# virajmehta/vae-training

Measured on AMD Instinct MI355X. Metric: ELBO train-step samples/sec, higher is better.
Workload: dtype f32; 1 GPU; M: linear-padding dd3 pad9 (D=12) L=20 linear enc/dec -tdv eps=-1 lr=1e-3 (seed_linpadding_expts.sh:1); batch_per_gpu=65536, global_batch=65536, data_dim=12, latent_dim=20, params=533, parallelism=dp1, grad_exchange=none, launch=direct library call x2395 steps (arguments marshalled once), input_batches=48

## Files before the change

vae_training_amd/csrc/linear_moments.hip:

```cpp
#include <stdlib.h>

#include <type_traits>

#include "comm_dev.h"
#include "rng_dev.h"
#include "vaek_internal.h"

namespace vaek {

using f32x4 = __attribute__((ext_vector_type(4))) float;
using d2 = __attribute__((ext_vector_type(2))) double;
typedef __attribute__((address_space(3))) void lds_void_t;
typedef const __attribute__((address_space(1))) void glb_void_t;

constexpr int LNT = 512, LNW = LNT / 64;
constexpr int kLinMaxPersist = 64;
constexpr int kLinReduceSets = 1;
constexpr int kLinReduceWgs = 24;

constexpr int kLinCommBanks = 4;
struct LinComm { unsigned long long* peer[kMaxWorld]; int world, rank, ng2; };

constexpr int kLinShards = 8, kLinShardStride = 32;
struct LinPtrs { const float* x[64]; const float* z1[64]; const float* z2[64]; };
struct LinArgs {
    int has_update, n_reduce, n_stream;
    int B, D, L, ntiles, T;
    const float* x; const float* z1; const float* z2; float* partial_out;
    const float* partial_in; double* M_out;
    const double* M_in;
    int persistent, n_steps, sets;
    float* partial_base; double* M_base;
    unsigned* cnt_stream; unsigned* cnt_reduce; unsigned* status;
    float* params; float* grads; float* m; float* v; int32_t* step_dev; float lr;
    float inv_bt, eps_cli, rows, rows_over_bt; int off_eps, P;
    float* loss_hist; long long loss_hist_cap;
    int stagger;
    LinComm comm;
};

#ifndef VAEK_LIN_ABL
#define VAEK_LIN_ABL 0
#endif
#ifdef VAEK_LIN_STAMPS
#ifdef VAEK_LIN_FOUR_BLOCK_TU
static __device__ unsigned long long* g_lin_stamp_buf = nullptr;
#else
__device__ unsigned long long* g_lin_stamp_buf = nullptr;
#endif
int lin_stamps_four(unsigned long long* buf);
#define LIN_STAMP(i)                                                                                         \
    do {                                                                                                     \
        if (VAEK_LIN_STAMPS == 2) break;          \
        __builtin_amdgcn_sched_barrier(0);                                                                   \
        unsigned long long _t;                                                                               \
        unsigned long long _r;                                                                               \
        asm volatile("s_waitcnt vmcnt(0) lgkmcnt(0)\n\ts_memtime %0\n\ts_memrealtime %1\n\ts_waitcnt lgkmcnt(0)" : "=s"(_t), "=s"(_r)::"memory"); \
        if (g_lin_stamp_buf && threadIdx.x == 0) { g_lin_stamp_buf[i] = _t; g_lin_stamp_buf[16 + (i)] = _r; } \
        __builtin_amdgcn_sched_barrier(0);                                                                   \
    } while (0)
#define LIN_NOW(v)                                                                                           \
    do {                                                                                                     \
        __builtin_amdgcn_sched_barrier(0);                                                                   \
        if (VAEK_LIN_STAMPS == 2) asm volatile("s_memrealtime %0\n\ts_waitcnt lgkmcnt(0)" : "=s"(v)::"memory");             \
        else asm volatile("s_waitcnt vmcnt(0) lgkmcnt(0)\n\ts_memrealtime %0\n\ts_waitcnt lgkmcnt(0)" : "=s"(v)::"memory"); \
        __builtin_amdgcn_sched_barrier(0);                                                                   \
    } while (0)
#define LIN_NOWQ(v)                                     \
    do {                                                                                                     \
        __builtin_amdgcn_sched_barrier(0);                                                                   \
        asm volatile("s_memrealtime %0\n\ts_waitcnt lgkmcnt(0)" : "=s"(v)::"memory");                        \
        __builtin_amdgcn_sched_barrier(0);                                                                   \
    } while (0)
#define LIN_PUT(i, v) do { if (g_lin_stamp_buf && threadIdx.x == 0) g_lin_stamp_buf[i] = (v); } while (0)
#define LIN_PUTMAX(i, v) do { if (g_lin_stamp_buf && threadIdx.x == 0) atomicMax(&g_lin_stamp_buf[i], (v)); } while (0)
#else
#define LIN_STAMP(i) do {} while (0)
#define LIN_NOW(v) do {} while (0)
#define LIN_NOWQ(v) do {} while (0)
#define LIN_PUT(i, v) do {} while (0)
#define LIN_PUTMAX(i, v) do {} while (0)
#endif

__device__ __forceinline__ void lin_glds16(const void* gsrc, void* lds_wave_base) {
    __builtin_amdgcn_global_load_lds((glb_void_t*)gsrc, (lds_void_t*)lds_wave_base, 16, 0, 0);
}
template <int N> __device__ __forceinline__ void lin_wait_vmcnt() { asm volatile("s_waitcnt vmcnt(%0)" ::"n"(N) : "memory"); }
__device__ __forceinline__ void lin_barrier() { asm volatile("s_waitcnt lgkmcnt(0)\n\ts_barrier" ::: "memory"); }
__device__ __forceinline__ void lin_wait_vmcnt_upto(int n) {
    switch (n) {
        case 1: lin_wait_vmcnt<1>(); break;   case 2: lin_wait_vmcnt<2>(); break;   case 3: lin_wait_vmcnt<3>(); break;
        case 4: lin_wait_vmcnt<4>(); break;   case 5: lin_wait_vmcnt<5>(); break;   case 6: lin_wait_vmcnt<6>(); break;
        case 7: lin_wait_vmcnt<7>(); break;   case 8: lin_wait_vmcnt<8>(); break;   case 9: lin_wait_vmcnt<9>(); break;
        case 10: lin_wait_vmcnt<10>(); break; case 11: lin_wait_vmcnt<11>(); break; case 12: lin_wait_vmcnt<12>(); break;
        case 13: lin_wait_vmcnt<13>(); break; case 14: lin_wait_vmcnt<14>(); break; case 15: lin_wait_vmcnt<15>(); break;
        case 16: lin_wait_vmcnt<16>(); break; case 17: lin_wait_vmcnt<17>(); break; case 18: lin_wait_vmcnt<18>(); break;
        case 19: lin_wait_vmcnt<19>(); break; case 20: lin_wait_vmcnt<20>(); break;
        default: lin_wait_vmcnt<0>(); break;
    }
}

__device__ __host__ constexpr int lin_blk(int NB, int b1, int b2) { return b1 * NB - b1 * (b1 - 1) / 2 + (b2 - b1); }

__device__ __forceinline__ void st_sc1(float* p, float v) { __hip_atomic_store(p, v, __ATOMIC_RELAXED, __HIP_MEMORY_SCOPE_AGENT); }
__device__ __forceinline__ void st_sc1(double* p, double v) { __hip_atomic_store(p, v, __ATOMIC_RELAXED, __HIP_MEMORY_SCOPE_AGENT); }
__device__ __forceinline__ float ld_sc1(const float* p) { return __hip_atomic_load(p, __ATOMIC_RELAXED, __HIP_MEMORY_SCOPE_AGENT); }
__device__ __forceinline__ double ld_sc1(const double* p) { return __hip_atomic_load(p, __ATOMIC_RELAXED, __HIP_MEMORY_SCOPE_AGENT); }

__device__ __forceinline__ void lin_wait_count(const unsigned* cnt, unsigned target, unsigned* status, unsigned tag) {
    if (threadIdx.x == 0) {
        unsigned spins = 0, seen;
        while ((seen = __hip_atomic_load(cnt, __ATOMIC_RELAXED, __HIP_MEMORY_SCOPE_AGENT)) < target) {
            __builtin_amdgcn_s_sleep(16);
            if ((++spins & 1023u) == 0) {
                if (__hip_atomic_load(status, __ATOMIC_RELAXED, __HIP_MEMORY_SCOPE_AGENT)) break;
                if (spins > (1u << 21)) {
                    unsigned expect = 0;
                    __hip_atomic_compare_exchange_strong(status, &expect, 0x80000000u | tag | (seen & 0xffffu), __ATOMIC_RELAXED,
                                                         __ATOMIC_RELAXED, __HIP_MEMORY_SCOPE_AGENT);
                    break;
                }
            }
        }
    }
    __syncthreads();
}

__device__ __forceinline__ void lin_wait_shards(const unsigned* cnt, unsigned target, unsigned* status, unsigned tag) {
    if (threadIdx.x == 0) {
        unsigned spins = 0, seen;
        for (;;) {
            unsigned v[kLinShards];
#pragma unroll
            for (int k = 0; k < kLinShards; ++k) v[k] = __hip_atomic_load(cnt + k * kLinShardStride, __ATOMIC_RELAXED, __HIP_MEMORY_SCOPE_AGENT);
            seen = 0;
#pragma unroll
            for (int k = 0; k < kLinShards; ++k) seen += v[k];
            if (seen >= target) break;
            __builtin_amdgcn_s_sleep(4);
            if ((++spins & 1023u) == 0) {
                if (__hip_atomic_load(status, __ATOMIC_RELAXED, __HIP_MEMORY_SCOPE_AGENT)) break;
                if (spins > (1u << 21)) {
                    unsigned expect = 0;
                    __hip_atomic_compare_exchange_strong(status, &expect, 0x80000000u | tag | (seen & 0xffffu), __ATOMIC_RELAXED,
                                                         __ATOMIC_RELAXED, __HIP_MEMORY_SCOPE_AGENT);
                    break;
                }
            }
        }
    }
    __syncthreads();
}

__device__ __forceinline__ double lin_sum_over_ranks(const LinComm& c, unsigned epoch, int o, double v, unsigned* status) {
    const unsigned long long bits = (unsigned long long)__double_as_longlong(v), tag = (unsigned long long)epoch << 32;
    const long long bank = (long long)(epoch & (kLinCommBanks - 1)) * c.world * c.ng2;
    for (int p = 0; p < c.world; ++p) {
        unsigned long long* q = c.peer[p] + bank + (long long)c.rank * c.ng2 + 2 * o;
        __hip_atomic_store(q, tag | (bits & 0xffffffffull), __ATOMIC_RELAXED, __HIP_MEMORY_SCOPE_SYSTEM);
        __hip_atomic_store(q + 1, tag | (bits >> 32), __ATOMIC_RELAXED, __HIP_MEMORY_SCOPE_SYSTEM);
    }
    const unsigned long long* own = c.peer[c.rank] + bank + 2 * o;
    double sum = 0.0;
    unsigned spins = 0;
    bool dead = false;
    for (int r = 0; r < c.world; ++r) {
        unsigned long long lo = 0, hi = 0;
        for (;;) {
            lo = __hip_atomic_load(own + (long long)r * c.ng2, __ATOMIC_RELAXED, __HIP_MEMORY_SCOPE_SYSTEM);
            hi = __hip_atomic_load(own + (long long)r * c.ng2 + 1, __ATOMIC_RELAXED, __HIP_MEMORY_SCOPE_SYSTEM);
            if (((unsigned)(lo >> 32) == epoch && (unsigned)(hi >> 32) == epoch) || dead) break;
            __builtin_amdgcn_s_sleep(8);
            if ((++spins & 1023u) == 0) {
                if (__hip_atomic_load(status, __ATOMIC_RELAXED, __HIP_MEMORY_SCOPE_AGENT)) dead = true;
                else if (spins > (1u << 21)) {
                    unsigned expect = 0;
                    __hip_atomic_compare_exchange_strong(status, &expect, 0x80000000u | (3u << 28) | ((unsigned)r << 16) | (epoch & 0xffffu),
                                                         __ATOMIC_RELAXED, __ATOMIC_RELAXED, __HIP_MEMORY_SCOPE_AGENT);
                    dead = true;
                }
            }
        }
        sum += __longlong_as_double((long long)((hi << 32) | (lo & 0xffffffffull)));
    }
// ... 1122 lines not shown
            double wsum = 0.0;
#pragma unroll
            for (int dt = 0; dt < PT; ++dt) {
                d4 C[2];
                double avk[KD], p1l[2][4], p1o[4], dw_sr[2], dw_br[2], dw_wr[KD][2], dw_dr[2][4];
                auto dw_s = [&](int ct) -> double& { return dw_sr[ct]; };
                auto dw_b = [&](int ct) -> double& { return dw_br[ct]; };
                auto dw_w = [&](int kk, int ct) -> double& { return dw_wr[kk][ct]; };
                auto dw_d = [&](int ct, int r) -> double& { return dw_dr[ct][r]; };
                const int d0 = 16 * dt;
#pragma unroll
                for (int ct = 0; ct < 2; ++ct) {
                    const int l = 16 * ct + j, lc = min(l, L - 1);
                    const double s_l = sd[lc], b_l = bed[lc];
                    dw_s(ct) = l < L ? s_l : 0.0; dw_b(ct) = l < L ? b_l : 0.0;
#pragma unroll
                    for (int kk = 0; kk < KD; ++kk) {
                        const int dd = 4 * kk + g;
                        const double w = Wed[min(dd, D - 1) * L + lc];
                        dw_w(kk, ct) = (dd < D && l < L) ? w : 0.0;
                    }
#pragma unroll
                    for (int r = 0; r < 4; ++r) dw_d(ct, r) = Wdd[lc * D + min(d0 + g + 4 * r, D - 1)];
                }
#pragma unroll
                for (int kk = 0; kk < KD; ++kk) avk[kk] = P1s[(d0 + j) * NFP + min(L + 4 * kk + g, NFP - 1)];
#pragma unroll
                for (int r = 0; r < 4; ++r) {
                    p1o[r] = P1s[(d0 + g + 4 * r) * NFP + fone];
#pragma unroll
                    for (int ct = 0; ct < 2; ++ct) p1l[ct][r] = P1s[(d0 + g + 4 * r) * NFP + min(16 * ct + j, L - 1)];
                }
                __builtin_amdgcn_sched_barrier(0);
#pragma unroll
                for (int ct = 0; ct < 2; ++ct) {
                    if (ct == 1 && RL1 == 0) continue;
                    const int l = 16 * ct + j;
#pragma unroll
                    for (int r = 0; r < 4; ++r) C[ct][r] = dw_s(ct) * p1l[ct][r] + dw_b(ct) * p1o[r];
#pragma unroll
                    for (int kk = 0; kk < KD; ++kk) C[ct] = __builtin_amdgcn_mfma_f64_16x16x4f64(avk[kk], dw_w(kk, ct), C[ct], 0, 0, 0);
#pragma unroll
                    for (int r = 0; r < 4; ++r) {
                        const int d = d0 + g + 4 * r;
                        if (l < L && d < D) { gq[off_wd + l * D + d] = c0 * C[ct][r]; wsum += dw_d(ct, r) * C[ct][r]; }
                    }
                }
            }
            wsum = lin_wave_sum(wsum);
            if (lane == 0) part[3 * NB] = wsum;
        }
        LIN_STAMP(4);
        __syncthreads();
        LIN_STAMP(5);
        const double rows = (double)a.rows;
        const float bc1 = (float)part[3 * NB + 4], bc2 = (float)part[3 * NB + 5];
#pragma unroll
        for (int k = 0; k < LKOUT; ++k) {
            const int idx = t + LNT * k;
            if (LNT * k >= P + 3) break;
            double gd = 0.0;
            if (idx < P && idx != off_eps) gd = gq[idx];
            else if (idx == off_eps || (idx >= P && idx < P + 3)) {
                double ssq = part[0], musq = part[1], z2r = part[2];
#pragma unroll
                for (int w = 1; w < NB; ++w) { ssq += part[3 * w]; musq += part[3 * w + 1]; z2r += part[3 * w + 2]; }
                ssq += part[3 * NB];
                const double klc = part[3 * NB + 3];
                if (idx == off_eps) gd = (double)a.eps_cli * (-0.5 * ssq * inv_var + 0.5 * rows * D + 0.5 * sigma * z2r * inv_var) * inv_bt;
                else {
                    const double dkl = (0.5 * musq - 0.5 * rows * klc) * inv_bt;
                    const double mse = (0.5 * ssq * inv_var + 0.5 * rows * D * ((double)kLog2Pi + eps)) * inv_bt;
                    gd = idx == P ? dkl + mse : (idx == P + 1 ? dkl : mse);
                }
            }
            const float gf = (float)gd;
            gout[k] = gf;
            if (idx == P && a.loss_hist) a.loss_hist[(long long)(tstep - 1) % a.loss_hist_cap] = gf;
            if (idx < P) adam_apply_f(pk(k), gf, mk(k), vk(k), a.lr, bc1, bc2);
        }
        LIN_STAMP(6);
    }
    __device__ __forceinline__ void store_state(const LinArgs& a, const float (&gout)[LKOUT], int tstep) {
        const int t = threadIdx.x;
#pragma unroll
        for (int k = 0; k < LKOUT; ++k) {
            const int idx = t + LNT * k;
            if (idx < P + kExtra) a.grads[idx] = gout[k];
            if (idx < P) { a.params[idx] = pk(k); a.m[idx] = mk(k); a.v[idx] = vk(k); }
        }
        if (t == 0) a.step_dev[0] = tstep;
    }
};

template <int NB, int DT, int LT>
using LinUpdMFor = std::conditional_t<NB == 3, LinUpdM<NB, DT, LT>, LinUpdMG<NB, DT, LT>>;

template <int NB, int DT, int LT>
__global__ __launch_bounds__(LNT) void lin_step_kernel(const LinArgs a) {
    extern __shared__ __attribute__((aligned(16))) char lin_smem[];
    const int b = blockIdx.x, t = threadIdx.x;
    constexpr int NO = NB * (NB + 1) / 2 * 256;
    if (b < a.has_update) {
        LinUpd<NB, DT, LT> u;
        u.carve(a, lin_smem);
        LIN_STAMP(0);
        const int tstep = a.step_dev[0] + 1;
        u.load_state(a);
        u.publish_params();
        u.template expand_M<false>(a.M_in);
        __syncthreads();
        float g[LKOUT];
        u.step(a, tstep, g);
        u.store_state(a, g, tstep);
        LIN_STAMP(7);
    } else if (b < a.has_update + a.n_reduce) {
        lin_reduce<false>(a.partial_in, a.M_out, a.ntiles, lin_smem, b - a.has_update, NO);
    } else {
        const int tile = b - a.has_update - a.n_reduce;
        const int wave = __builtin_amdgcn_readfirstlane(t >> 6), lane = t & 63;
        const LinTile tl(a.D, a.L, a.T);
        const int stride = max(tl.bytes, lin_scratch_bytes(NB)), v_off = stride, c_off = v_off + 4 * a.T;
        for (int p = wave; p < tl.np; p += LNW) lin_issue_piece(a, tl, a.x, a.z1, a.z2, tile, p, lin_smem, lane);
        lin_write_vcol(reinterpret_cast<float*>(lin_smem + v_off), a.T, (int)min((long long)a.T, (long long)a.B - (long long)tile * a.T), t);
        if (t == 0) *reinterpret_cast<float*>(lin_smem + c_off) = 0.f;
        lin_wait_vmcnt<0>();
        lin_barrier();
        lin_fix_ragged(a, tl, a.x, a.z1, a.z2, tile, lin_smem, t);
        f32x4 acc[NB * (NB + 1) / 2];
        lin_tile_products<NB, 0, LNW>(a, tl, lin_smem, 0, v_off, c_off, acc, lane, wave, [](int) {});
        lin_barrier();
        lin_tile_combine<NB, false, LNW>(acc, lin_smem, a.partial_out + (long long)tile * NO, t, wave, lane);
    }
}

template <int NB, int DT, int LT, int JT, bool GEN>
__global__ __launch_bounds__(LNT, 2) void lin_persist_kernel(const LinArgs a, const std::conditional_t<GEN, BatchArgs, LinPtrs> src) {
    extern __shared__ __attribute__((aligned(16))) char lin_smem[];
    const int b = blockIdx.x, t = threadIdx.x, N = a.n_steps;
    constexpr int NO = NB * (NB + 1) / 2 * 256;
    const int per_set = a.n_reduce / a.sets;
    if (b < a.has_update) {
        LinUpdMFor<NB, DT, LT> u;
        u.carve(a, lin_smem);
        int tstep = a.step_dev[0];
        u.load_state(a);
        float g[LKOUT];
#pragma unroll
        for (int k = 0; k < LKOUT; ++k) g[k] = 0.f;
        constexpr int NM = LinUpdMFor<NB, DT, LT>::NM;
        double mreg[NM], mnext[NM];
        bool have_next = false;
        LIN_STAMP(10);
        for (int n = 0; n < N; ++n) {
            LIN_STAMP(0);
            u.publish_params(a);
            LIN_STAMP(9);
            if (!have_next) {
                lin_wait_count(a.cnt_reduce + n, (unsigned)per_set, a.status, (1u << 28) | ((unsigned)n << 16));
                if (t < 64 * NB) u.fetch_M(a.M_base + (long long)n * NO, mreg);
            } else {
                __syncthreads();
#pragma unroll
                for (int k = 0; k < NM; ++k) mreg[k] = mnext[k];
            }
            LIN_STAMP(8);
            ++tstep;
            u.step(a, tstep, mreg, g, n + 1 < N ? a.cnt_reduce + n + 1 : nullptr, (unsigned)per_set, a.M_base + (long long)(n + 1) * NO, mnext, have_next);
            LIN_STAMP(7);
            { [[maybe_unused]] unsigned long long te = 0; LIN_NOWQ(te); LIN_PUT(64 + n, te); }
        }
        u.store_state(a, g, tstep);
        for (int k = t; k < N * kLinShards; k += LNT) __hip_atomic_store(a.cnt_stream + k * kLinShardStride, 0u, __ATOMIC_RELAXED, __HIP_MEMORY_SCOPE_AGENT);
        for (int k = t; k < N; k += LNT) __hip_atomic_store(a.cnt_reduce + k, 0u, __ATOMIC_RELAXED, __HIP_MEMORY_SCOPE_AGENT);
    } else if (b < a.has_update + a.n_reduce) {
        const int rb = b - a.has_update, set = rb / per_set, ro = rb % per_set;
        const int tstep0 = a.step_dev[0];
        [[maybe_unused]] unsigned long long r0 = 0, r1 = 0, r2 = 0, racc_w = 0, racc_r = 0;
        for (int n = set; n < N; n += a.sets) {
            LIN_NOWQ(r0);
            lin_wait_shards(a.cnt_stream + n * kLinShards * kLinShardStride, (unsigned)a.ntiles, a.status, (2u << 28) | ((unsigned)n << 16));
            LIN_NOWQ(r1);
            for (int sub = ro; sub < NO / 32; sub += 2 * per_set) {
                if (sub != ro) __syncthreads();
                const float* pin = a.partial_base + (long long)n * a.ntiles * NO;
                const unsigned epoch = (unsigned)(tstep0 + n + 1);
                if (sub + per_set < NO / 32)
                    lin_reduce_pair(pin, a.M_base + (long long)n * NO, a.ntiles, lin_smem, sub, sub + per_set, NO, a.comm, epoch, a.status);
                else lin_reduce<true>(pin, a.M_base + (long long)n * NO, a.ntiles, lin_smem, sub, NO, &a.comm, epoch, a.status);
            }
            lin_wait_vmcnt<0>();
            __syncthreads();
            LIN_NOWQ(r2);
            racc_w += r1 - r0; racc_r += r2 - r1;
            if (rb == 5) { LIN_PUT(40, racc_w); LIN_PUT(41, racc_r); }
            if (rb == 5 && n < 3) { LIN_PUT(56 + 2 * n, r1); LIN_PUT(57 + 2 * n, r2); }
            if (t == 0) __hip_atomic_fetch_add(a.cnt_reduce + n, 1u, __ATOMIC_RELAXED, __HIP_MEMORY_SCOPE_AGENT);
            { [[maybe_unused]] unsigned long long te = 0; LIN_NOW(te); LIN_PUTMAX(128 + n, te); }
        }
    } else {
        const int sid = b - a.has_update - a.n_reduce, S = a.n_stream;
        { [[maybe_unused]] unsigned long long te = 0; LIN_NOWQ(te); if (sid == 0) LIN_PUT(50, te); if (sid == S / 2) LIN_PUT(51, te); if (sid == S - 1) LIN_PUT(52, te); }
        const int wave = __builtin_amdgcn_readfirstlane(t >> 6), lane = t & 63;
        const LinTile tl(a.D, a.L, a.T);
        const int stride = max(tl.bytes, lin_ring_scratch_bytes(NB));
        const int v_off = 3 * stride, vr_off = v_off + 4 * a.T, c_off = vr_off + 4 * a.T;
        const float** tab = reinterpret_cast<const float**>(lin_smem + c_off + 16);
        if constexpr (!GEN) {
            if (t < 3 * kLinMaxPersist) {
                const int which = t / kLinMaxPersist, n = t % kLinMaxPersist;
                tab[t] = n < N ? (which == 0 ? src.x : which == 1 ? src.z1 : src.z2)[n] : nullptr;
            }
        }
        [[maybe_unused]] float* const Amat = reinterpret_cast<float*>(lin_smem + c_off + 16);
        if constexpr (GEN) {
            if (src.kind == 0 && t < src.dd * src.did) Amat[t] = src.A[t];
        }
        const int valid_last = a.B - (a.ntiles - 1) * a.T;
        lin_write_vcol(reinterpret_cast<float*>(lin_smem + v_off), a.T, a.T, t);
        lin_write_vcol(reinterpret_cast<float*>(lin_smem + vr_off), a.T, valid_last, t);
        if (t == 0) { *reinterpret_cast<float*>(lin_smem + c_off) = 0.f; *reinterpret_cast<unsigned*>(lin_smem + c_off + 8) = 0u; }
        __syncthreads();
        const int per_batch = sid < a.ntiles ? (a.ntiles - sid + S - 1) / S : 0, items = N * per_batch;
        const bool loader = wave >= kLinCW;
        const int lw = wave - kLinCW;
        constexpr int NLW = LNW - kLinCW;
        auto share = [&](int n) { return lw < n ? (n - lw + NLW - 1) / NLW : 0; };
        const int npw = (GEN || !loader) ? 0 : share(tl.nz1) + share(tl.nx) + share(tl.np - tl.nz1 - tl.nx);
        const int sw = wave < (NO / 4 + 63) / 64 ? 1 : 0;
        struct Pos {
            int idx, n, r, slot;
            __device__ __forceinline__ void advance(int per_batch) { ++idx; slot = slot == 2 ? 0 : slot + 1; if (++r == per_batch) { r = 0; ++n; } }
        };
        auto pos_tile = [&](const Pos& q) { return sid + q.r * S; };
        Pos p_cur{0, 0, 0, 0}, p_load{0, 0, 0, 0}, p_sig{0, 0, 0, 0};
        LinTileSrc nxt;
        nxt.on = false;
        auto prepare = [&]() __attribute__((always_inline)) {
            if constexpr (!GEN) {
                nxt.on = false;
                if (p_load.idx < items) {
                    const int n = p_load.n;
                    nxt.prepare(a, tab[n], tab[kLinMaxPersist + n], tab[2 * kLinMaxPersist + n], pos_tile(p_load), lin_smem + p_load.slot * stride);
                }
                p_load.advance(per_batch);
            }
        };
        auto issue_pieces = [&]() __attribute__((always_inline)) {
            if constexpr (!GEN) { if (!(VAEK_LIN_ABL & 8) && nxt.on) nxt.issue_tile(tl, lw, NLW, lane); }
        };
        constexpr int GT = NLW * 64;
        [[maybe_unused]] const int gD = DT ? DT : a.D, gL = LT ? LT : a.L, nzb = (gL + gD + 3) / 4;
        [[maybe_unused]] const int nlat = a.T * nzb, xr = (a.T + GT - 1) / GT, npair = nlat / (2 * GT), rem = nlat - 2 * GT * npair;
        [[maybe_unused]] const int gen_rounds = xr + npair + (rem + GT - 1) / GT;
        [[maybe_unused]] const unsigned step0 = (unsigned)a.step_dev[0];
        [[maybe_unused]] int g_kind = 0, g_dd = 0, g_did = 0; [[maybe_unused]] float g_noise = 0.f; [[maybe_unused]] unsigned g_tag = 0;
        if constexpr (GEN) { g_kind = src.kind; g_dd = src.dd; g_did = src.did; g_noise = src.noise_std; g_tag = src.tag; }
        auto gen_round = [&](const Pos& q, int k, int gt) __attribute__((always_inline)) {
            if constexpr (GEN) {
                if (q.idx < items && k < gen_rounds) {
                    const uint2 key = make_uint2((unsigned)src.seed, (unsigned)(src.seed >> 32));
                    const long long row_lo = (long long)pos_tile(q) * a.T;
                    const unsigned step = step0 + (unsigned)q.n;
                    char* slot = lin_smem + q.slot * stride;
                    auto put = [&](int z, const float (&n4)[4]) __attribute__((always_inline)) {
                        const int r = z / nzb, q = z - r * nzb, c0 = 4 * q;
                        const bool live = row_lo + r < a.B;
                        const f32x4 v4 = live ? f32x4{n4[0], n4[1], n4[2], n4[3]} : f32x4{0.f, 0.f, 0.f, 0.f};
                        float* z1r = reinterpret_cast<float*>(slot) + r * gL;
                        float* z2r = reinterpret_cast<float*>(slot + tl.oZ2) + r * gD;
                        if (c0 + 3 < gL && gL % 4 == 0) *reinterpret_cast<f32x4*>(z1r + c0) = v4;
                        else if (c0 >= gL && (c0 - gL) + 3 < gD && gD % 4 == 0 && gL % 4 == 0) *reinterpret_cast<f32x4*>(z2r + (c0 - gL)) = v4;
                        else {
#pragma unroll
                            for (int c = 0; c < 4; ++c) {
                                if (c0 + c < gL) z1r[c0 + c] = v4[c];
                                else if (c0 + c < gL + gD) z2r[c0 + c - gL] = v4[c];
                            }
                        }
                    };
                    auto draw = [&](int z, float (&n4)[4]) __attribute__((always_inline)) {
                        const int r = z / nzb;
                        latent_block(src, step, src.row0 + row_lo + r, key, z - r * nzb, n4);
                    };
                    if (k >= xr && k < xr + npair) {
                        const int za = 2 * GT * (k - xr) + gt;
                        float na[4], nb[4];
                        draw(za, na); draw(za + GT, nb);
                        put(za, na); put(za + GT, nb);
                    } else if (k >= xr + npair) {
                        const int z = 2 * GT * npair + GT * (k - xr - npair) + gt;
                        if (z < nlat) {
                            float n4[4];
                            draw(z, n4);
                            put(z, n4);
                        }
                    } else {
                        const int row = gt + GT * k;
                        if (row < a.T) {
                            const long long lrow = row_lo + row, grow = src.row0 + lrow;
                            const bool live = lrow < a.B;
                            float nrm[16];
                            dataset_normals(src, step, grow, key, nrm);
                            float* xr_ = reinterpret_cast<float*>(slot + tl.oX) + row * gD;
                            float inv = 0.f;
                            if (g_kind == 2) {
                                float nsq = 0.f;
#pragma unroll
                                for (int d = 0; d < 16; ++d) if (d < g_dd) nsq = fmaf(nrm[d], nrm[d], nsq);
                                inv = 1.f / sqrtf(nsq);
                            }
                            for (int c0 = 0; c0 < gD; c0 += 4) {
                                float o[4] = {0.f, 0.f, 0.f, 0.f};
                                if (c0 < g_dd) {
#pragma unroll
                                    for (int c = 0; c < 4; ++c) {
                                        const int d = c0 + c;
                                        float v = 0.f;
                                        if (d < g_dd) {
                                            if (g_kind == 0) {
#pragma unroll
                                                for (int kk = 0; kk < 16; ++kk) if (kk < g_did) v = fmaf(Amat[d * g_did + kk], nrm[kk], v);
                                            } else {
#pragma unroll
                                                for (int kk = 0; kk < 16; ++kk) v = (kk == d) ? nrm[kk] : v;
                                                v *= inv;
                                            }
                                        }
                                        o[c] = v;
                                    }
                                }
                                if (g_kind == 0 && g_noise > 0.f) {
                                    float n4[4];
                                    normals4(philox4x32_10(make_uint4((unsigned)grow, (unsigned)((g_did + 3) / 4 + c0 / 4), step, g_tag), key), n4);
#pragma unroll
                                    for (int c = 0; c < 4; ++c) o[c] = fmaf(g_noise, n4[c], o[c]);
                                }
                                const f32x4 v4 = live ? f32x4{o[0], o[1], o[2], o[3]} : f32x4{0.f, 0.f, 0.f, 0.f};
                                if (gD % 4 == 0) *reinterpret_cast<f32x4*>(xr_ + c0) = v4;
                                else {
#pragma unroll
                                    for (int c = 0; c < 4; ++c) if (c0 + c < gD) xr_[c0 + c] = v4[c];
                                }
                            }
                        }
                    }
                }
            }
        };
        [[maybe_unused]] unsigned* const ticket = reinterpret_cast<unsigned*>(lin_smem + c_off + 8);
        auto gen_share = [&](const Pos& q0, const Pos& q1, int nitems) __attribute__((always_inline)) {
            if constexpr (GEN) {
                const unsigned units = (unsigned)gen_rounds * NLW, total = units * (unsigned)nitems;
#pragma unroll 1
                for (;;) {
                    unsigned u = 0;
                    if (lane == 0) u = __hip_atomic_fetch_add(ticket, 1u, __ATOMIC_RELAXED, __HIP_MEMORY_SCOPE_WORKGROUP);
                    u = (unsigned)__builtin_amdgcn_readfirstlane((int)u);
                    if (u >= total) break;
                    const bool second = u >= units;
                    const unsigned v = second ? u - units : u;
                    gen_round(second ? q1 : q0, (int)(v / NLW), (int)(v % NLW) * 64 + lane);
                }
            }
        };
        unsigned* const my_shard = a.cnt_stream + (b & (kLinShards - 1)) * kLinShardStride;
        auto signal = [&]() {
            if (t == 0) __hip_atomic_fetch_add(my_shard + p_sig.n * kLinShards * kLinShardStride, 1u, __ATOMIC_RELAXED, __HIP_MEMORY_SCOPE_AGENT);
            p_sig.advance(per_batch);
        };
        if constexpr (GEN) {
            Pos q1 = p_load;
            q1.advance(per_batch);
            gen_share(p_load, q1, 2);
            p_load.advance(per_batch); p_load.advance(per_batch);
            lin_barrier();
            if (t == 0) *ticket = 0u;
        } else if (loader) {
            prepare();
            issue_pieces();
            prepare();
            issue_pieces();
        }
        [[maybe_unused]] unsigned long long s0 = 0, s1 = 0, s2 = 0, s3 = 0, s4 = 0, s5 = 0, s6 = 0, sacc_i = 0, sacc_l = 0, sacc_f = 0, sacc_m = 0, sacc_p = 0, sacc_b = 0;
        for (int i = 0; i < items; ++i) {
            LIN_NOWQ(s0);
            lin_wait_vmcnt_upto((i + 1 < items ? npw : 0) + (i >= 1 ? sw : 0));
            LIN_NOWQ(s1);
            lin_barrier();
            LIN_NOWQ(s2);
            if (i >= 3) signal();
            const int n = p_cur.n, tile = pos_tile(p_cur), slot_off = p_cur.slot * stride;
            char* slot = lin_smem + slot_off;
            const bool ragged = tile == a.ntiles - 1 && valid_last < a.T;
            if constexpr (!GEN) {
                if (ragged) lin_fix_ragged(a, tl, tab[n], tab[kLinMaxPersist + n], tab[2 * kLinMaxPersist + n], tile, slot, t);
            }
            LIN_NOWQ(s3);
            f32x4 acc[NB * (NB + 1) / 2];
            if (!loader) lin_tile_products<NB, JT, kLinCW>(a, tl, lin_smem, slot_off, ragged ? vr_off : v_off, c_off, acc, lane, wave, [](int) {});
            if constexpr (GEN) {
                gen_share(p_load, p_load, 1);
                p_load.advance(per_batch);
            } else if (loader && i > 0) {
                prepare();
                issue_pieces();
            }
            LIN_NOWQ(s5);
            lin_barrier();
            if constexpr (GEN) { if (t == 0) *ticket = 0u; }
            LIN_NOWQ(s6);
            lin_tile_combine<NB, true, kLinCW>(acc, slot, a.partial_base + ((long long)n * a.ntiles + tile) * NO, t, wave, lane);
            if (i == 0) {
                lin_wait_vmcnt<0>();
                lin_barrier();
                signal();
                if (sid == 0) { [[maybe_unused]] unsigned long long te = 0; LIN_NOWQ(te); LIN_PUT(53, te); }
                if constexpr (!GEN) {
                    if (loader) {
                        prepare();
                        issue_pieces();
                    }
                }
            }
            LIN_NOWQ(s4);
            if (i + 1 < items) { sacc_i += s1 - s0; sacc_l += s2 - s1; sacc_f += s3 - s2; sacc_m += s4 - s3; sacc_p += s5 - s3; sacc_b += s6 - s5; }
            if (sid == 7) { LIN_PUT(42, sacc_i); LIN_PUT(43, sacc_l); LIN_PUT(44, sacc_f); LIN_PUT(45, sacc_m); LIN_PUT(46, (unsigned long long)items); LIN_PUT(47, sacc_p); LIN_PUT(48, sacc_b); }
            p_cur.advance(per_batch);
        }
        lin_wait_vmcnt<0>();
        lin_barrier();
        if (items - 2 >= 1) signal();
        if (items - 1 >= 1) signal();
    }
}

constexpr unsigned kLinMagic = 0x4c494e33u;
#ifndef VAEK_LIN_FOUR_BLOCK_TU
__global__ void lin_init_kernel(unsigned* cnt, int n_words, unsigned* status) {
    for (int k = threadIdx.x; k < n_words; k += blockDim.x) cnt[k] = 0u;
    if (threadIdx.x == 0 && status[1] != kLinMagic) { status[0] = 0u; status[1] = kLinMagic; }
}
#endif

typedef void (*LinPersistKernel)(const LinArgs, const LinPtrs);
typedef void (*LinPersistGenKernel)(const LinArgs, const BatchArgs);
LinPersistKernel lin_persist_four(int which);
LinPersistGenKernel lin_persist_four_gen(int which);

#ifndef VAEK_LIN_FOUR_BLOCK_TU
constexpr size_t kLinMaxLds = 160 * 1024;
constexpr size_t kLinCntStreamBytes = (size_t)kLinMaxPersist * kLinShards * kLinShardStride * 4, kLinCntBytes = kLinCntStreamBytes + 1024, kLinHeadBytes = kLinCntBytes + 256;

LinPlan lin_plan(const vaek_ctx* c) {
    LinPlan p{};
    const int D = c->D, L = c->L;
    p.ok = c->cfg.n_enc_hidden == 0 && c->cfg.n_dec_hidden == 0 && !c->cfg.sigmoid_decoder && c->cfg.dtype == VAEK_F32 &&
           L + 2 * D + 1 <= 64 && (long long)c->B * std::min(D, L) >= 8;
    if (!p.ok) return p;
    p.NB = (L + 2 * D + 1 + 15) / 16 <= 3 ? 3 : 4;
    p.NO = p.NB * (p.NB + 1) / 2 * 256;
    const auto slot_bytes = [&](int T) { return std::max((size_t)LinTile(D, L, T).bytes, (size_t)lin_scratch_bytes(p.NB)); };
    const auto ring_slot_bytes = [&](int T) { return std::max((size_t)LinTile(D, L, T).bytes, (size_t)lin_ring_scratch_bytes(p.NB)); };
    const auto ring_bytes = [&](int T) { return 3 * ring_slot_bytes(T) + 8 * (size_t)T + 16 + 3 * kLinMaxPersist * sizeof(void*) + 64; };
    const auto ksteps_ok = [&](int T) { return (LinTile(D, L, T).np + LNW - kLinCW - 1) / (LNW - kLinCW) <= 18; };
    const int smax = c->n_cu - 1 - kLinReduceSets * kLinReduceWgs;
    const bool upd_ok = p.NB == 3 ? LinUpdM<3, 0, 0>::shape_ok(D, L) : LinUpdMG<4, 0, 0>::shape_ok(D, L);
    p.T = 256;
    if (p.NB == 3) {
        if (smax >= 16 && c->B > 256 * smax) {
            const int T = 32 * (int)(((long long)c->B + 32ll * smax - 1) / (32ll * smax));
            if (T <= 512 && ksteps_ok(T) && ring_bytes(T) <= kLinMaxLds) p.T = T;
        }
    } else if (upd_ok && smax >= 16) {
        int T = 256;
        while (T > 32 && !(ksteps_ok(T) && ring_bytes(T) <= kLinMaxLds)) T -= 32;
        p.T = T;
    }
    p.ntiles = (c->B + p.T - 1) / p.T;
    const size_t upd = std::max(p.NB == 3 ? LinUpd<3, 0, 0>::lds_bytes(D, L) : LinUpd<4, 0, 0>::lds_bytes(D, L),
                                p.NB == 3 ? LinUpdM<3, 0, 0>::lds_bytes(D, L, (int)c->P) : LinUpdMG<4, 0, 0>::lds_bytes(D, L, (int)c->P));
    p.lds_step = std::max(slot_bytes(p.T) + 4 * (size_t)p.T + 16, std::max(upd, (size_t)2 * 16 * 32 * sizeof(double))) + 64;
    p.lds_persist = std::max(std::max(p.lds_step, ring_bytes(p.T)), (size_t)82 * 1024);
    p.persist = upd_ok && p.lds_persist <= kLinMaxLds && ksteps_ok(p.T) && smax >= 16;
    if (p.persist) {
        const int per = (p.ntiles + smax - 1) / smax;
        p.n_stream = (p.ntiles + per - 1) / per;
        p.n_reduce = kLinReduceSets * std::min(kLinReduceWgs, p.NO / 32);
    }
    p.which_persist = p.NB == 3 ? (D == 12 && L == 20 && p.T == 288 ? 0 : 1) : (D == 20 && L == 20 && p.T == 192 ? 3 : 2);
    p.which_step = D == 12 && L == 20 ? 2 : p.NB - 3;
    const int slots = p.persist ? kLinMaxPersist : 2;
    p.M_off = kLinHeadBytes;
    p.partial_off = p.M_off + (size_t)slots * p.NO * sizeof(double) + 256;
    p.ws_bytes = (p.partial_off + (size_t)slots * p.ntiles * p.NO * sizeof(float) + 256 + 255) / 256 * 256;
    if (c->cfg.world > 1 && p.persist) p.comm_bytes = (size_t)kLinCommBanks * c->cfg.world * 2 * p.NO * sizeof(unsigned long long);
    return p;
}

bool lin_steps_supported(const vaek_ctx* c) {
    return c->lin.ok && (c->cfg.world == 1 || (c->lin.persist && c->comm.ready && c->comm.lin_bytes > 0));
}
bool lin_steps_gen_supported(const vaek_ctx* c, int kind) { return lin_steps_supported(c) && c->lin.persist && (kind == 0 || kind == 2); }

struct LinWs { float* partial; double* M; unsigned* cnt; unsigned* cnt_reduce; unsigned* status; };
static LinWs lin_ws(const vaek_ctx* c, void* ws) {
    char* base = static_cast<char*>(ws) + c->ws_lin;
    LinWs w;
    w.cnt = reinterpret_cast<unsigned*>(base); w.cnt_reduce = reinterpret_cast<unsigned*>(base + kLinCntStreamBytes);
    w.status = reinterpret_cast<unsigned*>(base + kLinCntBytes);
    w.M = reinterpret_cast<double*>(base + c->lin.M_off); w.partial = reinterpret_cast<float*>(base + c->lin.partial_off);
    return w;
}

typedef void (*LinStepKernel)(const LinArgs);
static const LinPersistKernel kLinPersist[] = {lin_persist_kernel<3, 12, 20, 18, false>, lin_persist_kernel<3, 0, 0, 0, false>,
                                                lin_persist_four(0), lin_persist_four(1)};
static const LinPersistGenKernel kLinPersistGen[] = {lin_persist_kernel<3, 12, 20, 18, true>, lin_persist_kernel<3, 0, 0, 0, true>,
                                                     lin_persist_four_gen(0), lin_persist_four_gen(1)};
static const LinStepKernel kLinStep[] = {lin_step_kernel<3, 0, 0>, lin_step_kernel<4, 0, 0>, lin_step_kernel<3, 12, 20>};
template <typename K, size_t N> static int lin_kernel(const K (&table)[N], int which, K* fn) {
    static thread_local PerDeviceOnce attr_set[N];
    if (attr_set[which].need()) {
        VAEK_HIP_CHECK(hipFuncSetAttribute((const void*)table[which], hipFuncAttributeMaxDynamicSharedMemorySize, (int)kLinMaxLds));
        attr_set[which].mark();
    }
    *fn = table[which];
    return VAEK_OK;
}

static void lin_fill_common(const vaek_ctx* c, LinArgs& a, float* params, float* grads, float* m, float* v, int32_t* step_dev, float lr) {
    a.B = c->B; a.D = c->D; a.L = c->L; a.T = c->lin.T; a.ntiles = c->lin.ntiles;
    a.params = params; a.grads = grads; a.m = m; a.v = v; a.step_dev = step_dev; a.lr = lr;
    const double rows = c->cfg.world > 1 ? (double)c->Bt : (double)c->B;
    a.inv_bt = (float)(1.0 / (double)c->Bt); a.eps_cli = c->cfg.eps_cli; a.rows = (float)rows;
    a.rows_over_bt = (float)(rows / (double)c->Bt); a.off_eps = (int)c->off_eps; a.P = (int)c->P;
    a.comm = LinComm{};
    a.comm.world = 1;
    if (c->cfg.world > 1 && c->comm.ready && c->comm.lin_bytes > 0) {
        a.comm.world = c->cfg.world; a.comm.rank = c->cfg.rank; a.comm.ng2 = 2 * c->lin.NO;
        for (int r = 0; r < c->cfg.world; ++r)
            a.comm.peer[r] = reinterpret_cast<unsigned long long*>(static_cast<char*>(c->comm.peers[r]) + c->comm.lin_off);
    }
    a.loss_hist = c->loss_hist; a.loss_hist_cap = c->loss_hist_cap;
    static const int stagger = getenv("VAEK_LIN_STAGGER") ? atoi(getenv("VAEK_LIN_STAGGER")) : 3;
    a.stagger = stagger;
}

static int lin_ensure_init(vaek_ctx* c, const LinWs& w, void* ws, hipStream_t st) {
    if (c->lin_ws_ready == ws) return VAEK_OK;
    hipStreamCaptureStatus cap = hipStreamCaptureStatusNone;
    VAEK_HIP_CHECK(hipStreamIsCapturing(st, &cap));
    hipLaunchKernelGGL(lin_init_kernel, dim3(1), dim3(1024), 0, st, w.cnt, (int)(kLinCntBytes / 4), w.status);
    VAEK_HIP_CHECK(hipGetLastError());
    c->lin_ws_issued = ws;
    c->lin_ws_ready = cap == hipStreamCaptureStatusNone ? ws : nullptr;
    return VAEK_OK;
}

static int lin_train_steps_impl(vaek_ctx* c, float* params, float* grads, float* m, float* v, int32_t* step_dev, const float* const* xs,
                                const float* const* z1s, const float* const* z2s, const BatchArgs* gen, int n_steps, float lr, void* ws, hipStream_t st) {
    const LinPlan& p = c->lin;
    const LinWs w = lin_ws(c, ws);
    static const char* env = getenv("VAEK_LIN_PERSIST");
    static const int roles = getenv("VAEK_LIN_ROLES") ? atoi(getenv("VAEK_LIN_ROLES")) : 7;
    const bool persistent = p.persist && (gen || c->cfg.world > 1 || !(env && atoi(env) == 0));
    if (gen && !persistent) { set_error("vaek_train_steps_gen: this context has no persistent form"); return VAEK_ERR_INVALID; }
    if (persistent) {
        LinPersistKernel fn = nullptr;
        LinPersistGenKernel fng = nullptr;
        if (int rc = gen ? lin_kernel(kLinPersistGen, p.which_persist, &fng) : lin_kernel(kLinPersist, p.which_persist, &fn)) return rc;
        if (int rc = lin_ensure_init(c, w, ws, st)) return rc;
        for (int s0 = 0; s0 < n_steps; s0 += kLinMaxPersist) {
            const int n = std::min(kLinMaxPersist, n_steps - s0);
            LinArgs a{};
            lin_fill_common(c, a, params, grads, m, v, step_dev, lr);
            a.persistent = 1; a.n_steps = n;
            a.sets = kLinReduceSets;
            a.has_update = 1; a.n_reduce = p.n_reduce; a.n_stream = p.n_stream;
            if (!(roles & 4)) a.has_update = 0;
            if (!(roles & 2)) { a.has_update = 0; a.n_reduce = 0; }
            if (!(roles & 1)) a.n_stream = 0;
            if (roles != 7) c->lin_ws_ready = nullptr;
            a.partial_base = w.partial; a.M_base = w.M;
            a.cnt_stream = w.cnt; a.cnt_reduce = w.cnt_reduce; a.status = w.status;
            const dim3 grid((unsigned)(a.has_update + a.n_reduce + a.n_stream));
            if (gen) {
                ProfScope ps("lin_moments_persistent_gen", st);
                launch_k(ps, fng, grid, dim3(LNT), p.lds_persist, st, a, *gen);
            } else {
                LinPtrs ptrs{};
                for (int i = 0; i < n; ++i) { ptrs.x[i] = xs[s0 + i]; ptrs.z1[i] = z1s[s0 + i]; ptrs.z2[i] = z2s[s0 + i]; }
                ProfScope ps("lin_moments_persistent", st);
                launch_k(ps, fn, grid, dim3(LNT), p.lds_persist, st, a, ptrs);
            }
        }
        VAEK_HIP_CHECK(hipGetLastError());
        return VAEK_OK;
    }
    LinStepKernel fn = nullptr;
    if (int rc = lin_kernel(kLinStep, p.which_step, &fn)) return rc;
    const size_t pstride = (size_t)p.ntiles * p.NO;
    for (int n = 0; n < n_steps + 2; ++n) {
        LinArgs a{};
        lin_fill_common(c, a, params, grads, m, v, step_dev, lr);
        a.has_update = (n >= 2 && (roles & 4)) ? 1 : 0;
        a.n_reduce = (n >= 1 && n <= n_steps && (roles & 2)) ? p.NO / 32 : 0;
        a.n_stream = (n < n_steps && (roles & 1)) ? p.ntiles : 0;
        if (a.has_update + a.n_reduce + a.n_stream == 0) continue;
        if (a.n_stream) { a.x = xs[n]; a.z1 = z1s[n]; a.z2 = z2s[n]; a.partial_out = w.partial + (n & 1) * pstride; }
        if (a.n_reduce) { a.partial_in = w.partial + ((n - 1) & 1) * pstride; a.M_out = w.M + ((n - 1) & 1) * p.NO; }
        a.M_in = w.M + (n & 1) * p.NO;
        ProfScope ps(a.n_stream ? "lin_moments_step" : "lin_moments_drain", st);
        launch_k(ps, fn, dim3((unsigned)(a.has_update + a.n_reduce + a.n_stream)), dim3(LNT), p.lds_step, st, a);
    }
    VAEK_HIP_CHECK(hipGetLastError());
    return VAEK_OK;
}

int lin_train_steps(vaek_ctx* c, float* params, float* grads, float* m, float* v, int32_t* step_dev, const float* const* xs,
                    const float* const* z1s, const float* const* z2s, int n_steps, float lr, void* ws, hipStream_t st) {
    return lin_train_steps_impl(c, params, grads, m, v, step_dev, xs, z1s, z2s, nullptr, n_steps, lr, ws, st);
}
int lin_train_steps_gen(vaek_ctx* c, float* params, float* grads, float* m, float* v, int32_t* step_dev, const BatchArgs& gen, int n_steps,
                        float lr, void* ws, hipStream_t st) {
    return lin_train_steps_impl(c, params, grads, m, v, step_dev, nullptr, nullptr, nullptr, &gen, n_steps, lr, ws, st);
}

int lin_moments(vaek_ctx* c, const float* x, const float* z1, const float* z2, double* M_out, void* ws, hipStream_t st) {
    const LinPlan& p = c->lin;
    LinStepKernel fn = nullptr;
    if (int rc = lin_kernel(kLinStep, p.which_step, &fn)) return rc;
    LinArgs a{};
    lin_fill_common(c, a, nullptr, nullptr, nullptr, nullptr, nullptr, 0.f);
    a.n_stream = p.ntiles; a.x = x; a.z1 = z1; a.z2 = z2; a.partial_out = lin_ws(c, ws).partial;
    { ProfScope ps("lin_moments_stream", st); launch_k(ps, fn, dim3((unsigned)p.ntiles), dim3(LNT), p.lds_step, st, a); }
    a.n_stream = 0; a.n_reduce = p.NO / 32; a.partial_in = a.partial_out; a.M_out = M_out;
    a.comm = LinComm{}; a.comm.world = 1;
    { ProfScope ps("lin_moments_reduce", st); launch_k(ps, fn, dim3((unsigned)a.n_reduce), dim3(LNT), p.lds_step, st, a); }
    VAEK_HIP_CHECK(hipGetLastError());
    return VAEK_OK;
}
int lin_update(vaek_ctx* c, float* params, float* grads, float* m, float* v, int32_t* step_dev, const double* M_in, float lr, hipStream_t st) {
    LinStepKernel fn = nullptr;
    if (int rc = lin_kernel(kLinStep, c->lin.which_step, &fn)) return rc;
    LinArgs a{};
    lin_fill_common(c, a, params, grads, m, v, step_dev, lr);
    a.has_update = 1; a.M_in = M_in;
    ProfScope ps("lin_moments_update", st);
    launch_k(ps, fn, dim3(1), dim3(LNT), c->lin.lds_step, st, a);
    VAEK_HIP_CHECK(hipGetLastError());
    return VAEK_OK;
}

int lin_steps_status(vaek_ctx* c, void* ws, int* gave_up) {
    *gave_up = 0;
    if (c->lin_ws_issued != ws) return VAEK_OK;
    const LinWs w = lin_ws(c, ws);
    unsigned s = 0;
    VAEK_HIP_CHECK(hipMemcpy(&s, w.status, sizeof(s), hipMemcpyDeviceToHost));
    *gave_up = (int)s;
    if (s) {
        VAEK_HIP_CHECK(hipMemset(w.status, 0, sizeof(unsigned)));
        c->lin_ws_ready = nullptr;
    }
    return VAEK_OK;
}

#endif

}

#if defined(VAEK_LIN_STAMPS) && !defined(VAEK_LIN_FOUR_BLOCK_TU)
extern "C" int vaek_debug_lin_stamps(unsigned long long* buf) {
    return hipMemcpyToSymbol(HIP_SYMBOL(vaek::g_lin_stamp_buf), &buf, sizeof(buf)) == hipSuccess ? vaek::lin_stamps_four(buf) : -2;
}
#endif
```

Before: 18.37 billion samples/s.

## Carry reduce and update stages across persistent launches via ring slots

Each persistent launch now streams steps s0..s1 while the reduce role trails by one step and the update role by two, with the leftover reduce/update work carried into the next launch through a ring of kLinSlots buffers. This is meant to remove the pipeline drain and fill at every 64-step launch boundary, so stream blocks of the next launch overlap with the tail reduce/update of the previous window. Counters, partials and M buffers are indexed by ring slot, and epoch/step offsets are adjusted. It adds index bookkeeping and relies on counters being reset correctly across launches.

```diff
diff --git a/vae_training_amd/csrc/linear_moments.hip b/vae_training_amd/csrc/linear_moments.hip
--- a/vae_training_amd/csrc/linear_moments.hip
+++ b/vae_training_amd/csrc/linear_moments.hip
@@ -15,6 +15,31 @@
 
 constexpr int LNT = 512, LNW = LNT / 64;
 constexpr int kLinMaxPersist = 64;
+constexpr int kLinCarry = 2, kLinSlots = kLinMaxPersist + kLinCarry;
+struct LinWindow { int first, count; };
+struct LinWindows { LinWindow stream, reduce, update; };
+constexpr LinWindows lin_windows(int K, int j) {
+    const int s0 = kLinMaxPersist * j, s1 = s0 + kLinMaxPersist < K ? s0 + kLinMaxPersist : K;
+    const bool last = s1 == K;
+    const int r0 = s0 >= 1 ? s0 - 1 : 0, u0 = s0 >= 2 ? s0 - 2 : 0;
+    return LinWindows{{s0, s1 - s0}, {r0, (last ? K : s1 - 1) - r0}, {u0, (last ? K : s1 - 2) - u0}};
+}
+constexpr int lin_launches(int K) { return (K + kLinMaxPersist - 1) / kLinMaxPersist; }
+constexpr bool lin_windows_ok(int K) {
+    int s = 0, r = 0, u = 0;
+    for (int j = 0; j < lin_launches(K); ++j) {
+        const LinWindows w = lin_windows(K, j);
+        if (w.stream.first != s || w.reduce.first != r || w.update.first != u) return false;
+        if (w.stream.count < 1 || w.stream.count > kLinMaxPersist || w.reduce.count < 1 || w.update.count < 1) return false;
+        s += w.stream.count; r += w.reduce.count; u += w.update.count;
+        if (r > s || u > r || s - w.update.first > kLinSlots) return false;
+    }
+    return s == K && r == K && u == K;
+}
+static_assert(lin_windows_ok(1) && lin_windows_ok(2) && lin_windows_ok(64) && lin_windows_ok(65) && lin_windows_ok(66) && lin_windows_ok(128) &&
+              lin_windows_ok(129) && lin_windows_ok(130) && lin_windows_ok(960), "launch windows of a vaek_train_steps call");
+static_assert(lin_windows(64, 0).update.count == 64 && lin_windows(130, 1).update.first == 62 && lin_windows(130, 1).reduce.first == 63 &&
+              lin_windows(130, 2).update.count == 4, "launch windows of a vaek_train_steps call");
 constexpr int kLinReduceSets = 1;
 constexpr int kLinReduceWgs = 24;
 
@@ -30,6 +55,8 @@
     const float* partial_in; double* M_out;
     const double* M_in;
     int persistent, n_steps, sets;
+    int n_red, n_str, slot_upd, slot_red, slot_str;
+    int d_red, d_str;
     float* partial_base; double* M_base;
     unsigned* cnt_stream; unsigned* cnt_reduce; unsigned* status;
     float* params; float* grads; float* m; float* v; int32_t* step_dev; float lr;
@@ -1458,13 +1485,15 @@
         double mreg[NM], mnext[NM];
         bool have_next = false;
         LIN_STAMP(10);
+        int sl = a.slot_upd;
         for (int n = 0; n < N; ++n) {
+            const int sl_next = sl + 1 == kLinSlots ? 0 : sl + 1;
             LIN_STAMP(0);
             u.publish_params(a);
             LIN_STAMP(9);
             if (!have_next) {
-                lin_wait_count(a.cnt_reduce + n, (unsigned)per_set, a.status, (1u << 28) | ((unsigned)n << 16));
-                if (t < 64 * NB) u.fetch_M(a.M_base + (long long)n * NO, mreg);
+                lin_wait_count(a.cnt_reduce + sl, (unsigned)per_set, a.status, (1u << 28) | ((unsigned)n << 16));
+                if (t < 64 * NB) u.fetch_M(a.M_base + (long long)sl * NO, mreg);
             } else {
                 __syncthreads();
 #pragma unroll
@@ -1472,28 +1501,39 @@
             }
             LIN_STAMP(8);
             ++tstep;
-            u.step(a, tstep, mreg, g, n + 1 < N ? a.cnt_reduce + n + 1 : nullptr, (unsigned)per_set, a.M_base + (long long)(n + 1) * NO, mnext, have_next);
+            u.step(a, tstep, mreg, g, n + 1 < N ? a.cnt_reduce + sl_next : nullptr, (unsigned)per_set, a.M_base + (long long)sl_next * NO, mnext, have_next);
             LIN_STAMP(7);
             { [[maybe_unused]] unsigned long long te = 0; LIN_NOWQ(te); LIN_PUT(64 + n, te); }
+            sl = sl_next;
         }
         u.store_state(a, g, tstep);
-        for (int k = t; k < N * kLinShards; k += LNT) __hip_atomic_store(a.cnt_stream + k * kLinShardStride, 0u, __ATOMIC_RELAXED, __HIP_MEMORY_SCOPE_AGENT);
-        for (int k = t; k < N; k += LNT) __hip_atomic_store(a.cnt_reduce + k, 0u, __ATOMIC_RELAXED, __HIP_MEMORY_SCOPE_AGENT);
+        for (int k = t; k < N * kLinShards; k += LNT) {
+            int s = a.slot_upd + k / kLinShards;
+            s = s >= kLinSlots ? s - kLinSlots : s;
+            __hip_atomic_store(a.cnt_stream + (s * kLinShards + k % kLinShards) * kLinShardStride, 0u, __ATOMIC_RELAXED, __HIP_MEMORY_SCOPE_AGENT);
+        }
+        for (int k = t; k < N; k += LNT) {
+            int s = a.slot_upd + k;
+            s = s >= kLinSlots ? s - kLinSlots : s;
+            __hip_atomic_store(a.cnt_reduce + s, 0u, __ATOMIC_RELAXED, __HIP_MEMORY_SCOPE_AGENT);
+        }
     } else if (b < a.has_update + a.n_reduce) {
         const int rb = b - a.has_update, set = rb / per_set, ro = rb % per_set;
         const int tstep0 = a.step_dev[0];
         [[maybe_unused]] unsigned long long r0 = 0, r1 = 0, r2 = 0, racc_w = 0, racc_r = 0;
-        for (int n = set; n < N; n += a.sets) {
+        int sl = a.slot_red + set;
+        sl = sl >= kLinSlots ? sl - kLinSlots : sl;
+        for (int n = set; n < a.n_red; n += a.sets, sl = sl + a.sets >= kLinSlots ? sl + a.sets - kLinSlots : sl + a.sets) {
             LIN_NOWQ(r0);
-            lin_wait_shards(a.cnt_stream + n * kLinShards * kLinShardStride, (unsigned)a.ntiles, a.status, (2u << 28) | ((unsigned)n << 16));
+            lin_wait_shards(a.cnt_stream + sl * kLinShards * kLinShardStride, (unsigned)a.ntiles, a.status, (2u << 28) | ((unsigned)n << 16));
             LIN_NOWQ(r1);
             for (int sub = ro; sub < NO / 32; sub += 2 * per_set) {
                 if (sub != ro) __syncthreads();
-                const float* pin = a.partial_base + (long long)n * a.ntiles * NO;
-                const unsigned epoch = (unsigned)(tstep0 + n + 1);
+                const float* pin = a.partial_base + (long long)sl * a.ntiles * NO;
+                const unsigned epoch = (unsigned)(tstep0 + a.d_red + n + 1);
                 if (sub + per_set < NO / 32)
-                    lin_reduce_pair(pin, a.M_base + (long long)n * NO, a.ntiles, lin_smem, sub, sub + per_set, NO, a.comm, epoch, a.status);
-                else lin_reduce<true>(pin, a.M_base + (long long)n * NO, a.ntiles, lin_smem, sub, NO, &a.comm, epoch, a.status);
+                    lin_reduce_pair(pin, a.M_base + (long long)sl * NO, a.ntiles, lin_smem, sub, sub + per_set, NO, a.comm, epoch, a.status);
+                else lin_reduce<true>(pin, a.M_base + (long long)sl * NO, a.ntiles, lin_smem, sub, NO, &a.comm, epoch, a.status);
             }
             lin_wait_vmcnt<0>();
             __syncthreads();
@@ -1501,8 +1541,8 @@
             racc_w += r1 - r0; racc_r += r2 - r1;
             if (rb == 5) { LIN_PUT(40, racc_w); LIN_PUT(41, racc_r); }
             if (rb == 5 && n < 3) { LIN_PUT(56 + 2 * n, r1); LIN_PUT(57 + 2 * n, r2); }
-            if (t == 0) __hip_atomic_fetch_add(a.cnt_reduce + n, 1u, __ATOMIC_RELAXED, __HIP_MEMORY_SCOPE_AGENT);
-            { [[maybe_unused]] unsigned long long te = 0; LIN_NOW(te); LIN_PUTMAX(128 + n, te); }
+            if (t == 0) __hip_atomic_fetch_add(a.cnt_reduce + sl, 1u, __ATOMIC_RELAXED, __HIP_MEMORY_SCOPE_AGENT);
+            { [[maybe_unused]] unsigned long long te = 0; LIN_NOW(te); LIN_PUTMAX(136 + n, te); }
         }
     } else {
         const int sid = b - a.has_update - a.n_reduce, S = a.n_stream;
@@ -1515,7 +1555,7 @@
         if constexpr (!GEN) {
             if (t < 3 * kLinMaxPersist) {
                 const int which = t / kLinMaxPersist, n = t % kLinMaxPersist;
-                tab[t] = n < N ? (which == 0 ? src.x : which == 1 ? src.z1 : src.z2)[n] : nullptr;
+                tab[t] = n < a.n_str ? (which == 0 ? src.x : which == 1 ? src.z1 : src.z2)[n] : nullptr;
             }
         }
         [[maybe_unused]] float* const Amat = reinterpret_cast<float*>(lin_smem + c_off + 16);
@@ -1527,7 +1567,7 @@
         lin_write_vcol(reinterpret_cast<float*>(lin_smem + vr_off), a.T, valid_last, t);
         if (t == 0) { *reinterpret_cast<float*>(lin_smem + c_off) = 0.f; *reinterpret_cast<unsigned*>(lin_smem + c_off + 8) = 0u; }
         __syncthreads();
-        const int per_batch = sid < a.ntiles ? (a.ntiles - sid + S - 1) / S : 0, items = N * per_batch;
+        const int per_batch = sid < a.ntiles ? (a.ntiles - sid + S - 1) / S : 0, items = a.n_str * per_batch;
         const bool loader = wave >= kLinCW;
         const int lw = wave - kLinCW;
         constexpr int NLW = LNW - kLinCW;
@@ -1535,11 +1575,14 @@
         const int npw = (GEN || !loader) ? 0 : share(tl.nz1) + share(tl.nx) + share(tl.np - tl.nz1 - tl.nx);
         const int sw = wave < (NO / 4 + 63) / 64 ? 1 : 0;
         struct Pos {
-            int idx, n, r, slot;
-            __device__ __forceinline__ void advance(int per_batch) { ++idx; slot = slot == 2 ? 0 : slot + 1; if (++r == per_batch) { r = 0; ++n; } }
+            int idx, n, r, slot, bs;
+            __device__ __forceinline__ void advance(int per_batch) {
+                ++idx; slot = slot == 2 ? 0 : slot + 1;
+                if (++r == per_batch) { r = 0; ++n; bs = bs == kLinSlots - 1 ? 0 : bs + 1; }
+            }
         };
         auto pos_tile = [&](const Pos& q) { return sid + q.r * S; };
-        Pos p_cur{0, 0, 0, 0}, p_load{0, 0, 0, 0}, p_sig{0, 0, 0, 0};
+        Pos p_cur{0, 0, 0, 0, a.slot_str}, p_load{0, 0, 0, 0, a.slot_str}, p_sig{0, 0, 0, 0, a.slot_str};
         LinTileSrc nxt;
         nxt.on = false;
         auto prepare = [&]() __attribute__((always_inline)) {
@@ -1559,7 +1602,7 @@
         [[maybe_unused]] const int gD = DT ? DT : a.D, gL = LT ? LT : a.L, nzb = (gL + gD + 3) / 4;
         [[maybe_unused]] const int nlat = a.T * nzb, xr = (a.T + GT - 1) / GT, npair = nlat / (2 * GT), rem = nlat - 2 * GT * npair;
         [[maybe_unused]] const int gen_rounds = xr + npair + (rem + GT - 1) / GT;
-        [[maybe_unused]] const unsigned step0 = (unsigned)a.step_dev[0];
+        [[maybe_unused]] const unsigned step0 = (unsigned)(a.step_dev[0] + a.d_str);
         [[maybe_unused]] int g_kind = 0, g_dd = 0, g_did = 0; [[maybe_unused]] float g_noise = 0.f; [[maybe_unused]] unsigned g_tag = 0;
         if constexpr (GEN) { g_kind = src.kind; g_dd = src.dd; g_did = src.did; g_noise = src.noise_std; g_tag = src.tag; }
         auto gen_round = [&](const Pos& q, int k, int gt) __attribute__((always_inline)) {
@@ -1672,7 +1715,7 @@
         };
         unsigned* const my_shard = a.cnt_stream + (b & (kLinShards - 1)) * kLinShardStride;
         auto signal = [&]() {
-            if (t == 0) __hip_atomic_fetch_add(my_shard + p_sig.n * kLinShards * kLinShardStride, 1u, __ATOMIC_RELAXED, __HIP_MEMORY_SCOPE_AGENT);
+            if (t == 0) __hip_atomic_fetch_add(my_shard + p_sig.bs * kLinShards * kLinShardStride, 1u, __ATOMIC_RELAXED, __HIP_MEMORY_SCOPE_AGENT);
             p_sig.advance(per_batch);
         };
         if constexpr (GEN) {
@@ -1716,7 +1759,7 @@
             lin_barrier();
             if constexpr (GEN) { if (t == 0) *ticket = 0u; }
             LIN_NOWQ(s6);
-            lin_tile_combine<NB, true, kLinCW>(acc, slot, a.partial_base + ((long long)n * a.ntiles + tile) * NO, t, wave, lane);
+            lin_tile_combine<NB, true, kLinCW>(acc, slot, a.partial_base + ((long long)p_cur.bs * a.ntiles + tile) * NO, t, wave, lane);
             if (i == 0) {
                 lin_wait_vmcnt<0>();
                 lin_barrier();
@@ -1738,6 +1781,7 @@
         lin_barrier();
         if (items - 2 >= 1) signal();
         if (items - 1 >= 1) signal();
+        { [[maybe_unused]] unsigned long long te = 0; LIN_NOWQ(te); LIN_PUTMAX(49, te); }
     }
 }
 
@@ -1756,7 +1800,8 @@
 
 #ifndef VAEK_LIN_FOUR_BLOCK_TU
 constexpr size_t kLinMaxLds = 160 * 1024;
-constexpr size_t kLinCntStreamBytes = (size_t)kLinMaxPersist * kLinShards * kLinShardStride * 4, kLinCntBytes = kLinCntStreamBytes + 1024, kLinHeadBytes = kLinCntBytes + 256;
+constexpr size_t kLinCntStreamBytes = (size_t)kLinSlots * kLinShards * kLinShardStride * 4, kLinCntBytes = kLinCntStreamBytes + 1024, kLinHeadBytes = kLinCntBytes + 256;
+static_assert(kLinSlots * sizeof(unsigned) <= 1024, "cnt_reduce");
 
 LinPlan lin_plan(const vaek_ctx* c) {
     LinPlan p{};
@@ -1796,7 +1841,7 @@
     }
     p.which_persist = p.NB == 3 ? (D == 12 && L == 20 && p.T == 288 ? 0 : 1) : (D == 20 && L == 20 && p.T == 192 ? 3 : 2);
     p.which_step = D == 12 && L == 20 ? 2 : p.NB - 3;
-    const int slots = p.persist ? kLinMaxPersist : 2;
+    const int slots = p.persist ? kLinSlots : 2;
     p.M_off = kLinHeadBytes;
     p.partial_off = p.M_off + (size_t)slots * p.NO * sizeof(double) + 256;
     p.ws_bytes = (p.partial_off + (size_t)slots * p.ntiles * p.NO * sizeof(float) + 256 + 255) / 256 * 256;
@@ -1877,11 +1922,14 @@
         LinPersistGenKernel fng = nullptr;
         if (int rc = gen ? lin_kernel(kLinPersistGen, p.which_persist, &fng) : lin_kernel(kLinPersist, p.which_persist, &fn)) return rc;
         if (int rc = lin_ensure_init(c, w, ws, st)) return rc;
-        for (int s0 = 0; s0 < n_steps; s0 += kLinMaxPersist) {
-            const int n = std::min(kLinMaxPersist, n_steps - s0);
+        for (int j = 0; j < lin_launches(n_steps); ++j) {
+            const LinWindows win = lin_windows(n_steps, j);
+            const int s0 = win.stream.first, n = win.stream.count;
             LinArgs a{};
             lin_fill_common(c, a, params, grads, m, v, step_dev, lr);
-            a.persistent = 1; a.n_steps = n;
+            a.persistent = 1; a.n_steps = win.update.count; a.n_red = win.reduce.count; a.n_str = n;
+            a.slot_upd = win.update.first % kLinSlots; a.slot_red = win.reduce.first % kLinSlots; a.slot_str = s0 % kLinSlots;
+            a.d_red = win.reduce.first - win.update.first; a.d_str = s0 - win.update.first;
             a.sets = kLinReduceSets;
             a.has_update = 1; a.n_reduce = p.n_reduce; a.n_stream = p.n_stream;
             if (!(roles & 4)) a.has_update = 0;
```

Measured after the change: 18.81 billion samples/s (median of 6 runs). 1.02x the previous value.
